# gue-ni/raytracer.glsl

Measured on AMD Instinct MI355X. Metric: Mpaths/s at 1920x1080, 8 bounces, 10k tris, higher is better.
Workload: dtype f32; 1 GPU; C2: 1920x1080, 8 bounces, 10000 triangles + 5 spheres, cube map 256^2, 1 spp/frame progressive, dof=1; parallelism=1 GPU(s), 8-row strips interleaved, gather to rank 0 every frame, frame_batch=1, kernel=4, wf_rays=4, wf_mode=1, wf_chunk=256, wf_early=0, wf_packed=0, mf_sets=4, mf_group_quads=32, mf_chunk_quads=32

## Files before the change

### raytracer.glsl_amd/csrc/rt_scan.hpp

```cpp
#pragma once
#include <type_traits>
#include "rt_mfma.hpp"

#pragma clang fp contract(off)

namespace rt {

typedef uint32_t u32x4 __attribute__((ext_vector_type(4)));
typedef float f32x6 __attribute__((ext_vector_type(6)));

template <bool kMax> __device__ __forceinline__ float half_reduce(float x)
{
    auto op = [](float a, float b) { return kMax ? __builtin_fmaxf(a, b) : __builtin_fminf(a, b); };
    auto dpp = [](float v, auto ctrl) { return __builtin_bit_cast(float, __builtin_amdgcn_update_dpp(0, __builtin_bit_cast(int, v), decltype(ctrl)::value, 0xf, 0xf, false)); };
    x = op(x, dpp(x, std::integral_constant<int, 0xB1>{}));
    x = op(x, dpp(x, std::integral_constant<int, 0x4E>{}));
    x = op(x, dpp(x, std::integral_constant<int, 0x141>{}));
    x = op(x, dpp(x, std::integral_constant<int, 0x140>{}));
    const float r0 = __builtin_bit_cast(float, __builtin_amdgcn_readlane(__builtin_bit_cast(int, x), 0));
    const float r1 = __builtin_bit_cast(float, __builtin_amdgcn_readlane(__builtin_bit_cast(int, x), 16));
    return op(r0, r1);
}
__device__ __forceinline__ float half_max(float x) { return half_reduce<true>(x); }
__device__ __forceinline__ float half_min(float x) { return half_reduce<false>(x); }
template <bool kMax> __device__ __forceinline__ float full_reduce(float x)
{
    auto op = [](float a, float b) { return kMax ? __builtin_fmaxf(a, b) : __builtin_fminf(a, b); };
    auto dpp = [](float v, auto ctrl) { return __builtin_bit_cast(float, __builtin_amdgcn_update_dpp(0, __builtin_bit_cast(int, v), decltype(ctrl)::value, 0xf, 0xf, false)); };
    x = op(x, dpp(x, std::integral_constant<int, 0xB1>{}));
    x = op(x, dpp(x, std::integral_constant<int, 0x4E>{}));
    x = op(x, dpp(x, std::integral_constant<int, 0x141>{}));
    x = op(x, dpp(x, std::integral_constant<int, 0x140>{}));
    auto rl = [&](int l) { return __builtin_bit_cast(float, __builtin_amdgcn_readlane(__builtin_bit_cast(int, x), l)); };
    return op(op(rl(0), rl(16)), op(rl(32), rl(48)));
}

constexpr uint32_t kCullRowWords = 128;
__device__ __forceinline__ void wave_lds_sync() { __builtin_amdgcn_fence(__ATOMIC_ACQ_REL, "wavefront"); __builtin_amdgcn_wave_barrier(); }
__device__ __forceinline__ bool cull_lane(const MfCull &c, bool have, const MfPacket &pk)
{
    bool skip = false, open = false;
    f3 W = mk(0.0f, 0.0f, 0.0f); float L = 0.0f, nz = 0.0f, Wn = 0.0f;
    if (have && c.Nmin > 0.0f) {
        const f3 gq = pk.O - mk(c.cx, c.cy, c.cz);
        L = __builtin_amdgcn_sqrtf(dot3(gq, gq)) * 1.0001f;
        nz = 9.5367431640625e-07f * __builtin_fmaf(c.lmax, pk.On, c.Pw) * 1.01f;
        W = cross3(pk.D, gq);
        Wn = __builtin_amdgcn_sqrtf(dot3(W, W));
        skip = mf_certified_ka(c, pk, gq, L, nz, Wn);
        open = !skip;
    }
    if (__any(open)) { if (open) skip = mf_certified_b(c, pk, W, L, nz, Wn); }
    return skip;
}

__global__ void __launch_bounds__(256) packet_cull_kernel(WaveBuffers wb, const MfCull *__restrict__ cull, uint32_t n_tiles, uint32_t bounce, float ro_add, float sigma_add,
                                                          const MfCull *__restrict__ node, uint32_t node_shift)
{
    __shared__ uint32_t s_row[4][kCullRowWords];
    __shared__ uint32_t s_open[4][64];
    const uint32_t n_rays = wb.counts[bounce];
    const RayQueue qin = (bounce & 1u) ? wb.q[1] : wb.q[0];
    const uint32_t lane = threadIdx.x & 63u, n_gran = (n_rays + 127u) / 128u;
    const float inf = __builtin_inff();
    for (uint32_t g = blockIdx.x * 4u + (threadIdx.x >> 6); g < n_gran; g += gridDim.x * 4u) {
        f3 o[2], dh[2]; bool valid[2]; bool usable = true;
        f3 olo = mk(inf, inf, inf), ohi = mk(-inf, -inf, -inf), dlo = olo, dhi = ohi;
#pragma unroll
        for (int k = 0; k < 2; ++k) {
            const uint32_t slot = g * 128u + (uint32_t)k * 64u + lane;
            valid[k] = slot < n_rays;
            o[k] = mk(0.0f, 0.0f, 0.0f); dh[k] = o[k];
            if (valid[k]) {
                const float4 a = qin.a[slot], b = qin.b[slot];
                o[k] = mk(a.x, a.y, a.z);
                const f3 d = mk(a.w, b.x, b.y);
                const float dd = dot3(d, d), il = __builtin_amdgcn_rsqf(dd), dl = dd * il;
                dh[k] = mk(d.x * il, d.y * il, d.z * il);
                usable &= (dl > 0.0f) && (dl < inf) && (fabsf(o[k].x) < 1e18f) && (fabsf(o[k].y) < 1e18f) && (fabsf(o[k].z) < 1e18f);
                olo = mk(fminf(olo.x, o[k].x), fminf(olo.y, o[k].y), fminf(olo.z, o[k].z)); ohi = mk(fmaxf(ohi.x, o[k].x), fmaxf(ohi.y, o[k].y), fmaxf(ohi.z, o[k].z));
                dlo = mk(fminf(dlo.x, dh[k].x), fminf(dlo.y, dh[k].y), fminf(dlo.z, dh[k].z)); dhi = mk(fmaxf(dhi.x, dh[k].x), fmaxf(dhi.y, dh[k].y), fmaxf(dhi.z, dh[k].z));
            }
        }
        olo = mk(full_reduce<false>(olo.x), full_reduce<false>(olo.y), full_reduce<false>(olo.z)); ohi = mk(full_reduce<true>(ohi.x), full_reduce<true>(ohi.y), full_reduce<true>(ohi.z));
        dlo = mk(full_reduce<false>(dlo.x), full_reduce<false>(dlo.y), full_reduce<false>(dlo.z)); dhi = mk(full_reduce<true>(dhi.x), full_reduce<true>(dhi.y), full_reduce<true>(dhi.z));
        MfPacket pk;
        pk.O = mk(0.5f * olo.x + 0.5f * ohi.x, 0.5f * olo.y + 0.5f * ohi.y, 0.5f * olo.z + 0.5f * ohi.z);
        f3 D = mk(0.5f * dlo.x + 0.5f * dhi.x, 0.5f * dlo.y + 0.5f * dhi.y, 0.5f * dlo.z + 0.5f * dhi.z);
        const float DD = dot3(D, D), iDl = __builtin_amdgcn_rsqf(DD), Dl = DD * iDl;
        pk.D = mk(D.x * iDl, D.y * iDl, D.z * iDl);
        float ro = 0.0f, sigma = 0.0f;
#pragma unroll
        for (int k = 0; k < 2; ++k)
            if (valid[k]) {
                const f3 eo = o[k] - pk.O, ed = dh[k] - pk.D;
                ro = fmaxf(ro, __builtin_amdgcn_sqrtf(dot3(eo, eo))); sigma = fmaxf(sigma, __builtin_amdgcn_sqrtf(dot3(ed, ed)));
            }
        pk.ro = full_reduce<true>(ro) * 1.0001f + 1e-30f + ro_add; pk.sigma = full_reduce<true>(sigma) * 1.0001f + 2e-6f + sigma_add;
        usable = !__any(!usable) && (Dl > 0.25f);
        pk.On = __builtin_amdgcn_sqrtf(dot3(pk.O, pk.O)) * 1.0001f + pk.ro;
        uint32_t *const row = wb.keep + (size_t)g * wb.keep_words;
        if (node_shift) {
            const uint32_t wv = threadIdx.x >> 6, S = 1u << node_shift, n_nodes = (n_tiles + S - 1u) >> node_shift;
            const uint32_t batch_nodes = (kCullRowWords * 32u) >> node_shift;
            const uint32_t grp = min(S, 32u);
            for (uint32_t b0 = 0; b0 < n_nodes; b0 += batch_nodes) {
                const uint32_t tile0 = b0 << node_shift, w0 = tile0 >> 5;
// ... 733 lines not shown
```

### raytracer.glsl_amd/csrc/rt_wavefront.hpp

```cpp
#pragma once
#include "rt_device.hpp"

#pragma clang fp contract(off)

namespace rt {

enum { kScalar = 0, kLds = 1 };
constexpr int kTile = 256;
constexpr int kBoundGroup = 64;

struct RayQueue {
    float4 *a;
    float4 *b;
    float4 *c;
    uint4 *rng;
    uint32_t *pixel;
};

struct WaveBuffers {
    RayQueue q[2];
    uint32_t *counts;
    float4 *sums;
    float4 *cam_a, *cam_b;
    uint4 *pix_rng;
    const float2 *group_bounds;
    unsigned long long *best[2];
    uint2 *cand;
    uint32_t *cand_counts;
    uint32_t cand_region;
    uint32_t *keep;
    uint32_t keep_words;
    uint32_t *items;
    uint32_t *item_counts;
    uint32_t items_stride;
    uint32_t hybrid_div;
    uint32_t *plan_prefix;
    uint32_t plan_stride;
    uint32_t *plan_total;
    unsigned long long *plan_base;
    uint32_t *sched;
    uint32_t sched_stride;
    uint32_t *cand_peak;
    RayQueue qt;
    uint2 *sort_kr;
    uint32_t *sort_hist;
    uint32_t *sort_hist_other;
    uint32_t sort_bits;
    uint32_t sort_ob;
    uint32_t sort_db, sort_T;
    float sort_lo[3], sort_inv_cell[3];
    float sort_in_lo[3], sort_in_hi[3];
    float sort_cen[3], sort_inv_unit;
    uint32_t sort_in_bits, sort_out_bits;
    uint32_t sort_in_order, sort_out_order;
    float4 *batch_rad;
    uint32_t batch_px;
};
constexpr uint32_t kBatchMax = 16u;
constexpr uint32_t kBatchPixelMask = 0x0FFFFFFFu;
struct BatchInfo { uint32_t n; int32_t frames[kBatchMax]; int32_t reset[kBatchMax]; };

struct PathState { f3 o, d, thr, rad; Rng rng; uint32_t pixel; };

typedef float rt_f4v __attribute__((ext_vector_type(4)));
typedef uint32_t rt_u4v __attribute__((ext_vector_type(4)));
typedef uint32_t rt_u2v __attribute__((ext_vector_type(2)));
__device__ __forceinline__ void store_through(float4 *p, float x, float y, float z, float w) { const rt_f4v v = {x, y, z, w}; asm volatile("global_store_dwordx4 %0, %1, off sc0 sc1\n\ts_nop 1" :: "v"(p), "v"(v) : "memory"); }
__device__ __forceinline__ void store_through(uint4 *p, uint32_t x, uint32_t y, uint32_t z, uint32_t w) { const rt_u4v v = {x, y, z, w}; asm volatile("global_store_dwordx4 %0, %1, off sc0 sc1\n\ts_nop 1" :: "v"(p), "v"(v) : "memory"); }
__device__ __forceinline__ void store_through(uint32_t *p, uint32_t x) { asm volatile("global_store_dword %0, %1, off sc0 sc1" :: "v"(p), "v"(x) : "memory"); }
__device__ __forceinline__ void store_through(unsigned long long *p, unsigned long long x) { const rt_u2v v = {(uint32_t)x, (uint32_t)(x >> 32)}; asm volatile("global_store_dwordx2 %0, %1, off sc0 sc1\n\ts_nop 1" :: "v"(p), "v"(v) : "memory"); }

__device__ __forceinline__ void store_ray(const RayQueue &q, uint32_t slot, const PathState &s, bool camera = false)
{
    store_through(q.a + slot, s.o.x, s.o.y, s.o.z, s.d.x);
    store_through(q.b + slot, s.d.y, s.d.z, s.thr.x, s.thr.y);
    if (!camera) store_through(q.c + slot, s.thr.z, s.rad.x, s.rad.y, s.rad.z);
    store_through(q.rng + slot, s.rng.x, s.rng.y, s.rng.z, s.rng.w);
// ... 504 lines not shown
    const float oa[3] = {o.x, o.y, o.z};
    const bool inside = o.x >= wb.sort_in_lo[0] && o.x <= wb.sort_in_hi[0] && o.y >= wb.sort_in_lo[1] && o.y <= wb.sort_in_hi[1] && o.z >= wb.sort_in_lo[2] && o.z <= wb.sort_in_hi[2];
    const uint32_t bits3 = inside ? wb.sort_in_bits : wb.sort_out_bits, order = inside ? wb.sort_in_order : wb.sort_out_order;
    uint32_t c[3], left[3];
#pragma unroll
    for (int a = 0; a < 3; ++a) {
        const uint32_t nb = (bits3 >> (4 * a)) & 15u;
        left[a] = nb;
        if (inside) c[a] = (uint32_t)fminf(fmaxf((oa[a] - wb.sort_lo[a]) * wb.sort_inv_cell[a], 0.0f), (float)((1u << nb) - 1u));
        else {
            const float u = fminf(fabsf(oa[a] - wb.sort_cen[a]) * wb.sort_inv_unit, 1.0e6f);
            const uint32_t j = min(7u, (__float_as_uint(1.0f + u) >> 23) - 127u);
            c[a] = (oa[a] >= wb.sort_cen[a] ? 8u + j : 7u - j) >> (4u - nb);
        }
    }
    uint32_t cell = 0u;
    const uint32_t n = left[0] + left[1] + left[2];
    for (uint32_t i = 0; i < n; ++i) {
        const uint32_t a = (order >> (2u * i)) & 3u;
        const uint32_t l = (a == 0u ? left[0] : a == 1u ? left[1] : left[2]) - 1u;
        const uint32_t v = a == 0u ? c[0] : a == 1u ? c[1] : c[2];
        cell = (cell << 1) | ((v >> l) & 1u);
        left[0] = a == 0u ? l : left[0]; left[1] = a == 1u ? l : left[1]; left[2] = a == 2u ? l : left[2];
    }
    return (dir << (T + 1u)) | (inside ? 0u : 1u << T) | (cell << (T - n));
}

template <bool kCount, bool kSort>
__global__ void __launch_bounds__(256) shade_kernel(SceneView sc, FrameParams P, ImageView im, WaveBuffers wb,
                                                    uint32_t bounce, uint4 *rng_out, Counters *counters)
{
    const uint32_t n_rays = wb.counts[bounce];
    const RayQueue qin = (bounce & 1u) ? wb.q[1] : wb.q[0];
    const RayQueue qout = kSort ? wb.qt : ((bounce & 1u) ? wb.q[0] : wb.q[1]);
    const unsigned long long *best_in = (bounce & 1u) ? wb.best[1] : wb.best[0];
    unsigned long long *best_out = (bounce & 1u) ? wb.best[0] : wb.best[1];
    const bool last_bounce = (bounce + 1u >= P.max_bounce);
    unsigned long long c_env = 0;
    __shared__ uint32_t s_cnt[5];
    for (uint32_t blk = blockIdx.x; blk * 256u < n_rays; blk += gridDim.x) {
    const uint32_t slot = blk * 256u + threadIdx.x;
    const bool valid = slot < n_rays;
    bool alive = false;
    PathState s;
    if (valid) {
        s = load_ray(qin, slot, bounce == 0u);
        const unsigned long long key = best_in[slot];
        Hit h; h.t = kInf; h.material = 0; h.point = h.normal = mk(0.0f, 0.0f, 0.0f);
        const bool hit_sphere = sphere_pass(sc, s.o, s.d, h);
        const bool hit_mesh = key != kNoHitKey;
        if (!hit_sphere && !hit_mesh) {
            f3 bg;
            if (P.use_envmap) { bg = env_lookup(sc, s.d); if (kCount) c_env++; }
            else bg = mk(P.background[0], P.background[1], P.background[2]);
            s.rad = s.rad + bg * s.thr;
        } else {
            const float mesh_t = hit_mesh ? __uint_as_float((uint32_t)(key >> 32)) : kInf;
            if (!(h.t < mesh_t)) {
                const TriPlane pl = sc.tri_planes[(uint32_t)key];
                h.t = mesh_t; h.point = s.o + s.d * mesh_t; h.normal = mk(pl.nx, pl.ny, pl.nz); h.material = pl.material;
            }
            alive = shade_hit(sc, h, s.rng, s.o, s.d, s.thr, s.rad) && !last_bounce;
        }
        if (!alive) finish_path(P, im, wb, s, rng_out);
    }
    const unsigned long long mask = __ballot(alive);
    const int lane = threadIdx.x & 63, wave = threadIdx.x >> 6;
    if (lane == 0) s_cnt[wave] = (uint32_t)__popcll(mask);
    __syncthreads();
    if (threadIdx.x == 0) {
        const uint32_t total = s_cnt[0] + s_cnt[1] + s_cnt[2] + s_cnt[3];
        s_cnt[4] = total ? atomicAdd(&wb.counts[bounce + 1u], total) : 0u;
    }
    __syncthreads();
    if (alive) {
        uint32_t wave_base = s_cnt[4];
        for (int w = 0; w < wave; ++w) wave_base += s_cnt[w];
        const uint32_t out_slot = wave_base + (uint32_t)__popcll(mask & ((1ull << lane) - 1ull));
        if (kSort) {
            const uint32_t key = ray_bin_key(wb, s.o, s.d);
            uint32_t grp_n = 1u, grp_rank = 0u; int grp_leader = lane;
            for (unsigned long long todo = __ballot(1); todo;) {
                const int l = __builtin_ctzll(todo);
                const uint32_t k0 = (uint32_t)__builtin_amdgcn_readlane((int)key, l);
                const unsigned long long m = __ballot(key == k0);
                if (key == k0) { grp_n = (uint32_t)__popcll(m); grp_rank = (uint32_t)__popcll(m & ((1ull << lane) - 1ull)); grp_leader = l; }
                todo &= ~m;
            }
            uint32_t base = 0u;
            if (lane == grp_leader) base = atomicAdd(wb.sort_hist + key, grp_n);
            const uint32_t rank = (uint32_t)__shfl((int)base, grp_leader) + grp_rank;
            store_ray(qout, out_slot, s);
            store_through(reinterpret_cast<unsigned long long *>(wb.sort_kr + out_slot), (unsigned long long)key | ((unsigned long long)rank << 32));
        } else { store_ray(qout, out_slot, s); store_through(best_out + out_slot, kNoHitKey); }
    }
    __syncthreads();
    }
    if (kCount) {
        atomicAdd(&counters->env_lookups, c_env);
        if (blockIdx.x == 0 && threadIdx.x == 0) atomicAdd(&counters->segments, (unsigned long long)n_rays);
    }
}

constexpr uint32_t kSortSeg = 4096;
__global__ void __launch_bounds__(256) sort_sums_kernel(WaveBuffers wb)
{
    __shared__ uint32_t part[4];
    const uint32_t *h = wb.sort_hist + (size_t)blockIdx.x * kSortSeg;
    const uint4 *h4 = reinterpret_cast<const uint4 *>(h);
    uint32_t s = 0;
#pragma unroll
    for (int k = 0; k < 4; ++k) { const uint4 v = h4[k * 256 + threadIdx.x]; s += v.x + v.y + v.z + v.w; }
    for (int off = 32; off > 0; off >>= 1) s += __shfl_xor(s, off);
    if ((threadIdx.x & 63u) == 0u) part[threadIdx.x >> 6] = s;
    __syncthreads();
    if (threadIdx.x == 0) store_through(wb.sort_hist + ((size_t)1u << wb.sort_bits) + blockIdx.x, part[0] + part[1] + part[2] + part[3]);
}
__global__ void __launch_bounds__(256) sort_prefix_kernel(WaveBuffers wb)
{
    __shared__ uint32_t part[4], wsum[4];
    const uint32_t *sums = wb.sort_hist + ((size_t)1u << wb.sort_bits);
    uint32_t before = 0;
    for (uint32_t i = threadIdx.x; i < blockIdx.x; i += 256u) before += sums[i];
    for (int off = 32; off > 0; off >>= 1) before += __shfl_xor(before, off);
    if ((threadIdx.x & 63u) == 0u) part[threadIdx.x >> 6] = before;
    __syncthreads();
    before = part[0] + part[1] + part[2] + part[3];
    uint32_t *h = wb.sort_hist + (size_t)blockIdx.x * kSortSeg + threadIdx.x * 16u;
    uint4 v[4];
#pragma unroll
    for (int k = 0; k < 4; ++k) v[k] = reinterpret_cast<const uint4 *>(h)[k];
    uint32_t c[16] = {v[0].x, v[0].y, v[0].z, v[0].w, v[1].x, v[1].y, v[1].z, v[1].w, v[2].x, v[2].y, v[2].z, v[2].w, v[3].x, v[3].y, v[3].z, v[3].w};
    uint32_t tot = 0;
#pragma unroll
    for (int k = 0; k < 16; ++k) { const uint32_t t = c[k]; c[k] = tot; tot += t; }
    uint32_t inc = tot;
    const uint32_t lane = threadIdx.x & 63u, wave = threadIdx.x >> 6;
    for (int off = 1; off < 64; off <<= 1) { const uint32_t t = __shfl_up(inc, off); if (lane >= (uint32_t)off) inc += t; }
    if (lane == 63u) wsum[wave] = inc;
    __syncthreads();
    uint32_t base = before + inc - tot;
    for (uint32_t w = 0; w < wave; ++w) base += wsum[w];
#pragma unroll
    for (int k = 0; k < 4; ++k) store_through(reinterpret_cast<uint4 *>(h) + k, base + c[4 * k], base + c[4 * k + 1], base + c[4 * k + 2], base + c[4 * k + 3]);
}
__global__ void __launch_bounds__(256) sort_scatter_kernel(WaveBuffers wb, uint32_t bounce)
{
    const uint32_t n_rays = wb.counts[bounce];
    const RayQueue qout = (bounce & 1u) ? wb.q[1] : wb.q[0];
    unsigned long long *best_out = (bounce & 1u) ? wb.best[1] : wb.best[0];
    {
        uint4 *const z = reinterpret_cast<uint4 *>(wb.sort_hist_other);
        const uint32_t n4 = (uint32_t)(((size_t)1u << wb.sort_bits) / 4u);
        for (uint32_t w = blockIdx.x * 256u + threadIdx.x; w < n4; w += gridDim.x * 256u) store_through(z + w, 0u, 0u, 0u, 0u);
    }
    for (uint32_t slot = blockIdx.x * 256u + threadIdx.x; slot < n_rays; slot += gridDim.x * 256u) {
        const uint2 kr = wb.sort_kr[slot];
        const uint32_t to = wb.sort_hist[kr.x] + kr.y;
        const float4 a = wb.qt.a[slot], b = wb.qt.b[slot], c = wb.qt.c[slot];
        const uint4 g = wb.qt.rng[slot];
        const uint32_t px = wb.qt.pixel[slot];
        if (to >= n_rays) { store_through(best_out + slot, kNoHitKey); continue; }
        store_through(qout.a + to, a.x, a.y, a.z, a.w);
        store_through(qout.b + to, b.x, b.y, b.z, b.w);
        store_through(qout.c + to, c.x, c.y, c.z, c.w);
        store_through(qout.rng + to, g.x, g.y, g.z, g.w);
        store_through(qout.pixel + to, px);
        store_through(best_out + slot, kNoHitKey);
    }
}

__global__ void __launch_bounds__(64) group_bounds_kernel(const TriEdges *__restrict__ edges, uint32_t n, float2 *__restrict__ out)
{
    const uint32_t g = blockIdx.x, v = g * kBoundGroup + threadIdx.x;
    float be = 0.0f, bm = 0.0f;
    if (v < n) { be = edges[v].bound_e; bm = edges[v].bound_m; }
    bool bad = !(be == be) || !(bm == bm);
#pragma unroll
    for (int off = 32; off > 0; off >>= 1) {
        be = fmaxf(be, __shfl_xor(be, off));
        bm = fmaxf(bm, __shfl_xor(bm, off));
    }
    if (__any(bad)) { be = __builtin_nanf(""); bm = __builtin_nanf(""); }
    if (threadIdx.x == 0) out[g] = make_float2(be, bm);
}

}
```

### raytracer.glsl_amd/csrc/rtgl_amd.hip

```cpp
#include <hip/hip_runtime.h>
#include <algorithm>
#include <cmath>
#include <cstdio>
#include <cstring>
#include <string>
#include <vector>
#include <map>
#include <mutex>
#include <thread>
#include <condition_variable>
#include <memory>

#include "../../include/rtgl_amd.h"
#include "rt_device.hpp"
#include "rt_wavefront.hpp"
#include "rt_mfma.hpp"
#include "rt_scan.hpp"

#pragma clang fp contract(off)

using namespace rt;


__global__ void __launch_bounds__(256) prepare_triangles_kernel(const float4 *__restrict__ vertices,
// ... 132 lines not shown
    std::vector<uint8_t> h_meshes, h_nodes, h_vertices;
    uint32_t n_meshes = 0, n_nodes = 0, n_vec4 = 0;

    SphereRec *d_spheres = nullptr; uint32_t n_spheres = 0;
    MaterialRec *d_materials = nullptr; uint32_t n_materials = 0;
    float4 *d_vertices = nullptr;
    uint32_t *d_sphere_visits = nullptr; uint32_t n_sphere_visits = 0;
    TriEdges *d_edges = nullptr; TriPlane *d_planes = nullptr; uint32_t n_tri_visits = 0;
    TriEdges *d_edges_s = nullptr; TriPlane *d_planes_s = nullptr;
    uint8_t *d_env = nullptr; int env_w = 0, env_h = 0, env_c = 0, env_faces = 0;
    float4 *d_image_own = nullptr, *d_image = nullptr;
    uint4 *d_rng = nullptr;
    Counters *d_counters = nullptr;
    uchar4 *d_u8 = nullptr;

    float2 *d_group_bounds = nullptr;
    MfGroup *d_mf_groups = nullptr; MfCull *d_mf_cull = nullptr; MfCull *d_mf_cull_node = nullptr; uint32_t cull_node_shift = 0; uint4 *d_mf_A = nullptr; uint32_t *d_mf_order = nullptr; uint32_t n_mf_groups = 0, mf_group_quads = 32; uint32_t *d_dbg_log = nullptr;
    void *d_wave = nullptr; size_t wave_capacity = 0; bool wave_multi = false;
    uint32_t *d_counts = nullptr; uint32_t counts_capacity = 0;
    uint32_t *h_counts = nullptr;
    hipEvent_t counts_ev = nullptr; bool counts_pending = false, counts_valid = false;
    bool timing_this_frame = false; uint32_t timing_frame_counter = 0;
    int kernel_in_use = -1;
    int n_cus = 256;
    uint2 *d_items = nullptr; size_t items_capacity = 0;
    uint32_t *d_sched = nullptr; size_t sched_capacity = 0;
    uint32_t *d_keep = nullptr; size_t keep_capacity = 0;
    uint32_t *d_keep0 = nullptr; size_t keep0_capacity = 0; bool keep0_valid = false; FrameParams keep0_params{}; uint32_t keep0_n0 = 0, keep0_words = 0; uint64_t keep0_scene = 0;
    uint64_t scene_version = 0;
    void *d_plan = nullptr; size_t plan_capacity = 0;
    void *d_stage = nullptr; size_t stage_capacity = 0;
    uint32_t *d_sort_hist = nullptr; uint32_t sort_bits_alloc = 0;
    int sort_set = 0; uint32_t sort_set_bits = 0; bool sort_sets_clean = false;
    float mesh_lo[3] = {0.0f, 0.0f, 0.0f}, mesh_hi[3] = {0.0f, 0.0f, 0.0f}, mesh_ext = 0.0f;
    uint2 *d_cand = nullptr; uint32_t cand_regions = 0, cand_region_pairs = 0, cand_region_target = 0; bool cand_fixed = false;
    bool solo_attr_set = false;
    bool group_explicit = false;
    bool kernel_explicit = false;
    uint32_t counts_n0 = 0, counts_len = 0;
    std::vector<uint32_t> est_counts;
    WaveBuffers wb{};

    std::vector<rtgl_context *> parts;
    std::vector<hipEvent_t> part_done;
    hipEvent_t gather_done = nullptr;
    std::vector<std::unique_ptr<PartWorker>> workers;
    bool gathered = false, peer_copy = true;

    std::vector<FrameParams> pending;
    float4 *d_batch_rad = nullptr; size_t batch_capacity = 0;
    uint32_t last_batch_frames = 1;
    bool tris_dirty = false, visits_dirty = false;
    FrameParams params{};
    bool have_params = false;
    int opt_kernel = RTGL_KERNEL_WAVEFRONT_MFMA_SOLO, opt_rng_state = 0, opt_counters = 0, opt_kernel_timing = 0, opt_wf_rays = 4, opt_wf_mode = kLds, opt_wf_chunk = 256, opt_wf_early = 0, opt_wf_packed = 0, opt_mf_chunk_quads = 32, opt_mf_group_quads = 32, opt_cull = 3, opt_sort_min_rays = 131072, opt_scan_waves = 0, opt_scan_dynamic = 0, opt_debug_skip_exact = 0, opt_frame_batch = 1;
};

static int fail(rtgl_context *ctx, int code, const std::string &msg)
{
    if (ctx) ctx->error = msg; else g_create_error = msg;
    return code;
}
#define HIPCHK(ctx, expr) do { hipError_t e_ = (expr); if (e_ != hipSuccess) \
    return fail(ctx, RTGL_ERR_DEVICE, std::string(#expr) + ": " + hipGetErrorString(e_)); } while (0)

template <typename T>
// ... 69 lines not shown
    *out = nullptr;
    if (width <= 0 || height <= 0 || world < 1 || rank < 0 || rank >= world || strip_rows <= 0 || (strip_rows % 8) != 0)
        return fail(nullptr, RTGL_ERR_INVALID, "rtgl_create: bad size / tiling arguments");
    int ndev = 0;
    if (hipGetDeviceCount(&ndev) != hipSuccess || ndev <= 0)
        return fail(nullptr, RTGL_ERR_NO_DEVICE, "no HIP device visible (this library has no CPU path)");
    if (device < 0 || device >= ndev) return fail(nullptr, RTGL_ERR_INVALID, "device ordinal out of range");
    rtgl_context *ctx = new rtgl_context();
    ctx->device = device; ctx->width = width; ctx->height = height;
    ctx->rank = rank; ctx->world = world; ctx->strip_rows = strip_rows;
    ctx->local_rows = local_rows_for(height, rank, world, strip_rows);
    auto bail = [&](int code) { g_create_error = ctx->error; rtgl_destroy(ctx); return code; };
#define CCHK(expr) do { hipError_t e_ = (expr); if (e_ != hipSuccess) { \
    ctx->error = std::string(#expr) + ": " + hipGetErrorString(e_); return bail(RTGL_ERR_DEVICE); } } while (0)
    CCHK(hipSetDevice(device));
    { hipDeviceProp_t prop; if (hipGetDeviceProperties(&prop, device) == hipSuccess && prop.multiProcessorCount > 0) ctx->n_cus = prop.multiProcessorCount; }
    CCHK(acquire_device_stream(device, &ctx->own_stream, &ctx->own_stream_shared));
    ctx->stream = ctx->own_stream;
    register_ctx_stream(ctx, device, ctx->stream);
    CCHK(hipEventCreate(&ctx->ev0));
    CCHK(hipEventCreate(&ctx->ev1));
    size_t img_bytes = (size_t)std::max(ctx->local_rows, 1) * width * sizeof(float4);
    CCHK(hipMalloc((void **)&ctx->d_image_own, img_bytes));
    CCHK(hipMemsetAsync(ctx->d_image_own, 0, img_bytes, ctx->stream));
    ctx->d_image = ctx->d_image_own;
    CCHK(hipMalloc((void **)&ctx->d_counters, 64));
    CCHK(hipMemsetAsync(ctx->d_counters, 0, 64, ctx->stream));
    CCHK(hipStreamSynchronize(ctx->stream));
#undef CCHK
    if (const char *k = getenv("RTGL_AMD_KERNEL")) { const int v = atoi(k); if (v >= RTGL_KERNEL_MEGA && v <= RTGL_KERNEL_WAVEFRONT_MFMA_SOLO && v != RTGL_KERNEL_REMOVED_3) { ctx->opt_kernel = v; ctx->kernel_explicit = true; } }
    if (const char *k = getenv("RTGL_AMD_SCAN_WAVES")) { const int v = atoi(k); if (v >= 0 && v <= 2) ctx->opt_scan_waves = v; }
    if (const char *k = getenv("RTGL_AMD_FRAME_BATCH")) { const int v = atoi(k); if (v >= 1 && v <= (int)kBatchMax) ctx->opt_frame_batch = v; }
    if (const char *k = getenv("RTGL_AMD_SCAN_DYNAMIC")) { const int v = atoi(k); if (v >= 0 && v <= 4) ctx->opt_scan_dynamic = v; }
    *out = ctx;
    return RTGL_OK;
}

static int flush_pending_noexcept(rtgl_context *ctx);
extern "C" int rtgl_create(rtgl_context **out, int width, int height, int device)
{
    return rtgl_create_tiled(out, width, height, device, 0, 1, 8);
}

extern "C" void rtgl_destroy(rtgl_context *ctx)
{
    if (!ctx) return;
    if (!ctx->pending.empty() && hipSetDevice(ctx->device) == hipSuccess && flush_pending_noexcept(ctx) != RTGL_OK)
        fprintf(stderr, "rtgl_destroy: %zu batched frame(s) could not be submitted: %s\n", ctx->pending.size(), ctx->error.c_str());
    unregister_ctx_stream(ctx);
    for (auto &w : ctx->workers) {
        { std::lock_guard<std::mutex> lk(w->m); w->state = PartWorker::kQuit; }
        w->cv.notify_all();
        if (w->th.joinable()) w->th.join();
    }
    ctx->workers.clear();
    for (rtgl_context *part : ctx->parts) rtgl_destroy(part);
    ctx->parts.clear();
    (void)hipSetDevice(ctx->device);
    for (hipEvent_t e : ctx->part_done) (void)hipEventDestroy(e);
    if (ctx->gather_done) (void)hipEventDestroy(ctx->gather_done);
    if (ctx->stream) (void)hipStreamSynchronize(ctx->stream);
#ifdef RT_SOLO_STAMPS
    if (ctx->d_dbg_log) {
        unsigned long long h[16 * 64];
        if (hipMemcpy(h, ctx->d_dbg_log, sizeof h, hipMemcpyDeviceToHost) == hipSuccess)
            for (int b = 0; b < 64 && h[16 * b + 8]; ++b) {
// ... 463 lines not shown
    const size_t local_px = (size_t)std::max(ctx->local_rows, 1) * ctx->width;
    if (ctx->opt_kernel == RTGL_KERNEL_WAVEFRONT_MFMA_SOLO) {
        const uint32_t need_regions = solo_regions(ctx);
        if (!ctx->cand_region_target) ctx->cand_region_target = std::max<uint32_t>(4096u, (uint32_t)std::min<uint64_t>(((uint64_t)n0 + need_regions - 1) / need_regions, 0xFFFFFFF0u));
        if (!ctx->d_cand || need_regions > ctx->cand_regions || ctx->cand_region_target > ctx->cand_region_pairs) {
            if (ctx->d_cand) { HIPCHK(ctx, hipFree(ctx->d_cand)); ctx->d_cand = nullptr; }
            ctx->cand_regions = need_regions; ctx->cand_region_pairs = ctx->cand_region_target;
            HIPCHK(ctx, hipMalloc((void **)&ctx->d_cand, ((size_t)need_regions * ctx->cand_region_pairs) * sizeof(uint2) + (size_t)need_regions * sizeof(uint32_t) + 256));
        }
        {
            const uint32_t real_quads = std::min(ctx->n_mf_groups * ctx->mf_group_quads, (ctx->n_tri_visits + (uint32_t)kMfQuadTris - 1) / (uint32_t)kMfQuadTris);
            ctx->wb.keep_words = std::max(1u, (real_quads * (uint32_t)kMfQuadTiles + 31u) / 32u);
            const size_t need = ((size_t)n0 / 128 + 16) * ctx->wb.keep_words;
            if (ctx->keep_capacity < need) {
                if (ctx->d_keep) { HIPCHK(ctx, hipFree(ctx->d_keep)); ctx->d_keep = nullptr; }
                HIPCHK(ctx, hipMalloc((void **)&ctx->d_keep, need * sizeof(uint32_t)));
                ctx->keep_capacity = need;
            }
        }
        ctx->wb.keep = ctx->d_keep;
        {
            ctx->wb.sched_stride = std::max<uint32_t>((uint32_t)ctx->n_cus, solo_chunks(ctx));
            const size_t need = (size_t)(max_bounce + 2) * ctx->wb.sched_stride;
            if (ctx->sched_capacity < need) {
                if (ctx->d_sched) { HIPCHK(ctx, hipFree(ctx->d_sched)); ctx->d_sched = nullptr; }
                HIPCHK(ctx, hipMalloc((void **)&ctx->d_sched, need * sizeof(uint32_t)));
                ctx->sched_capacity = need;
            }
            ctx->wb.sched = ctx->d_sched;
        }
        if (ctx->opt_cull == 3) {
            if (ctx->stage_capacity < n0) {
                if (ctx->d_stage) { HIPCHK(ctx, hipFree(ctx->d_stage)); ctx->d_stage = nullptr; }
                HIPCHK(ctx, hipMalloc(&ctx->d_stage, (size_t)n0 * 76 + 1024));
                ctx->stage_capacity = n0;
            }
            uint8_t *p = (uint8_t *)ctx->d_stage;
            const size_t cap = ctx->stage_capacity;
            ctx->wb.qt.a = (float4 *)p; p += cap * 16; ctx->wb.qt.b = (float4 *)p; p += cap * 16; ctx->wb.qt.c = (float4 *)p; p += cap * 16;
            ctx->wb.qt.rng = (uint4 *)p; p += cap * 16; ctx->wb.sort_kr = (uint2 *)p; p += cap * 8; ctx->wb.qt.pixel = (uint32_t *)p;
            ctx->wb.sort_ob = n0 > (12u << 20) ? 5u : 4u;
            if (const char *e = getenv("RTGL_AMD_SORT_OB")) { const int v = atoi(e); if (v >= 1 && v <= 5) ctx->wb.sort_ob = (uint32_t)v; }
            ctx->wb.sort_db = 4u;
            if (const char *e = getenv("RTGL_AMD_SORT_DB")) { const int v = atoi(e); if (v >= 2 && v <= 6) ctx->wb.sort_db = (uint32_t)v; }
            ctx->wb.sort_bits = 8u + 3u * ctx->wb.sort_ob;
            ctx->wb.sort_T = ctx->wb.sort_bits - 1u - 2u * ctx->wb.sort_db;
            if (ctx->sort_bits_alloc < ctx->wb.sort_bits) {
                if (ctx->d_sort_hist) { HIPCHK(ctx, hipFree(ctx->d_sort_hist)); ctx->d_sort_hist = nullptr; }
                const size_t bins = (size_t)1 << ctx->wb.sort_bits;
                HIPCHK(ctx, hipMalloc((void **)&ctx->d_sort_hist, 2 * (bins + bins / kSortSeg) * sizeof(uint32_t)));
                ctx->sort_bits_alloc = ctx->wb.sort_bits; ctx->sort_sets_clean = false;
            }
            ctx->wb.sort_hist = ctx->d_sort_hist; ctx->wb.sort_hist_other = ctx->d_sort_hist;
            set_bin_cells(ctx);
        }
        ctx->wb.hybrid_div = 3u;
        if (const char *e = getenv("RTGL_AMD_HYBRID_DIV")) { const int v = atoi(e); if (v >= 1 && v <= 64) ctx->wb.hybrid_div = (uint32_t)v; }
        ctx->wb.items = reinterpret_cast<uint32_t *>(ctx->d_items); ctx->wb.item_counts = reinterpret_cast<uint32_t *>(ctx->d_items);
        ctx->wb.cand = ctx->d_cand;
        ctx->wb.cand_counts = reinterpret_cast<uint32_t *>(ctx->d_cand + (size_t)ctx->cand_regions * ctx->cand_region_pairs);
        ctx->wb.cand_region = ctx->cand_region_pairs;
        if (const char *cc = getenv("RTGL_DEBUG_CAND_CAP")) { ctx->wb.cand_region = std::min<uint32_t>(ctx->wb.cand_region, (uint32_t)atoi(cc)); ctx->cand_fixed = true; }
    }
    if (ctx->wave_capacity < n0 || (multi_sample && !ctx->wave_multi)) {
        if (ctx->d_wave) { HIPCHK(ctx, hipFree(ctx->d_wave)); ctx->d_wave = nullptr; }
        size_t q_bytes = (size_t)n0 * (68 + 8), bytes = 2 * q_bytes + 1024 + (multi_sample ? local_px * 64 : 0);
        HIPCHK(ctx, hipMalloc(&ctx->d_wave, bytes));
        ctx->wave_capacity = n0; ctx->wave_multi = multi_sample;
        uint8_t *p = (uint8_t *)ctx->d_wave;
        for (int q = 0; q < 2; ++q) {
            ctx->wb.q[q].a = (float4 *)p; p += (size_t)n0 * 16;
            ctx->wb.q[q].b = (float4 *)p; p += (size_t)n0 * 16;
            ctx->wb.q[q].c = (float4 *)p; p += (size_t)n0 * 16;
// ... 104 lines not shown
    MfView mf{ctx->d_mf_groups, ctx->n_mf_groups, gq, n_quads, ctx->d_mf_A, ctx->d_dbg_log, ctx->d_mf_cull, ctx->d_edges_s, ctx->d_planes_s, ctx->d_mf_order};
    if (!ctx->solo_attr_set) {
        for (const void *fn : {reinterpret_cast<const void *>(&scan_solo_kernel<false, 1, 0>), reinterpret_cast<const void *>(&scan_solo_kernel<true, 1, 0>),
                               reinterpret_cast<const void *>(&scan_solo_kernel<false, 2, 0>), reinterpret_cast<const void *>(&scan_solo_kernel<true, 2, 0>),
                               reinterpret_cast<const void *>(&scan_solo_kernel<false, 1, 1>), reinterpret_cast<const void *>(&scan_solo_kernel<true, 1, 1>),
                               reinterpret_cast<const void *>(&scan_solo_kernel<false, 2, 1>), reinterpret_cast<const void *>(&scan_solo_kernel<true, 2, 1>),
                               reinterpret_cast<const void *>(&scan_solo_kernel<false, 1, 2>), reinterpret_cast<const void *>(&scan_solo_kernel<true, 1, 2>),
                               reinterpret_cast<const void *>(&scan_solo_kernel<false, 2, 2>), reinterpret_cast<const void *>(&scan_solo_kernel<true, 2, 2>),
                               reinterpret_cast<const void *>(&scan_solo_kernel<false, 1, 3>), reinterpret_cast<const void *>(&scan_solo_kernel<true, 1, 3>),
                               reinterpret_cast<const void *>(&scan_solo_kernel<false, 2, 3>), reinterpret_cast<const void *>(&scan_solo_kernel<true, 2, 3>)}) {
            hipFuncAttributes fattr;
            HIPCHK(ctx, hipFuncGetAttributes(&fattr, fn));
            HIPCHK(ctx, hipFuncSetAttribute(fn, hipFuncAttributeMaxDynamicSharedMemorySize, (int)(160 * 1024 - fattr.sharedSizeBytes)));
        }
        ctx->solo_attr_set = true;
    }

    if (cull) {
        float ro_add = 0.0f, sigma_add = 0.0f;
        bool have_bits = false;
        if (bounce == 0 && cam && camera_keep_widening(*cam, &ro_add, &sigma_add) && !getenv("RTGL_AMD_NO_CAMERA_KEEP")) {
            const size_t need = ((size_t)n0 / 128 + 16) * ctx->wb.keep_words;
            if (ctx->keep0_capacity < need) {
                if (ctx->d_keep0) { HIPCHK(ctx, hipFree(ctx->d_keep0)); ctx->d_keep0 = nullptr; }
                HIPCHK(ctx, hipMalloc((void **)&ctx->d_keep0, need * sizeof(uint32_t)));
                ctx->keep0_capacity = need; ctx->keep0_valid = false;
            }
            have_bits = ctx->keep0_valid && ctx->keep0_n0 == n0 && ctx->keep0_words == ctx->wb.keep_words && ctx->keep0_scene == ctx->scene_version && same_camera(ctx->keep0_params, *cam);
            ctx->wb.keep = ctx->d_keep0;
            if (!have_bits) { ctx->keep0_valid = true; ctx->keep0_n0 = n0; ctx->keep0_words = ctx->wb.keep_words; ctx->keep0_scene = ctx->scene_version; ctx->keep0_params = *cam; }
        } else { ctx->wb.keep = ctx->d_keep; ro_add = sigma_add = 0.0f; }
        if (!have_bits)
        hipLaunchKernelGGL(packet_cull_kernel, dim3(std::max(1u, std::min((est_gran + 3u) / 4u, 8192u))), dim3(256), 0, ctx->stream, ctx->wb, ctx->d_mf_cull, real_quads * (uint32_t)kMfQuadTiles, bounce, ro_add, sigma_add,
                           ctx->d_mf_cull_node, ctx->d_mf_cull_node ? ctx->cull_node_shift : 0u);
        if (dist == 2) {
            const uint32_t stride = n0 / Cfg::kRaysPerWave + 1u;
            const size_t off_tot = (((size_t)chunks * stride * sizeof(uint32_t)) + 255) & ~(size_t)255, off_base = (off_tot + (size_t)chunks * sizeof(uint32_t) + 255) & ~(size_t)255;
            const size_t need = off_base + ((size_t)chunks + 1) * sizeof(unsigned long long);
            if (ctx->plan_capacity < need) {
                if (ctx->d_plan) { HIPCHK(ctx, hipFree(ctx->d_plan)); ctx->d_plan = nullptr; }
                HIPCHK(ctx, hipMalloc(&ctx->d_plan, need));
                ctx->plan_capacity = need;
            }
            ctx->wb.plan_prefix = reinterpret_cast<uint32_t *>(ctx->d_plan); ctx->wb.plan_stride = stride;
            ctx->wb.plan_total = reinterpret_cast<uint32_t *>(reinterpret_cast<uint8_t *>(ctx->d_plan) + off_tot);
            ctx->wb.plan_base = reinterpret_cast<unsigned long long *>(reinterpret_cast<uint8_t *>(ctx->d_plan) + off_base);
            if (ctx->opt_counters) hipLaunchKernelGGL(scan_plan_kernel<true>, dim3(chunks), dim3(256), 0, ctx->stream, ctx->wb, bounce, chunk_quads, real_quads, ctx->d_counters);
            else hipLaunchKernelGGL(scan_plan_kernel<false>, dim3(chunks), dim3(256), 0, ctx->stream, ctx->wb, bounce, chunk_quads, real_quads, ctx->d_counters);
            hipLaunchKernelGGL(scan_plan_base_kernel, dim3(1), dim3(64), 0, ctx->stream, ctx->wb, chunks);
        }
        if (dynamic) {
        const uint32_t stride = n0 / Cfg::kRaysPerWave + 1u;
        const size_t head = ((size_t)ctx->wb.sched_stride * sizeof(uint32_t) + 255) & ~(size_t)255, need = head + (size_t)chunks * stride * sizeof(uint32_t);
        if (ctx->items_capacity < need) {
            if (ctx->d_items) { HIPCHK(ctx, hipFree(ctx->d_items)); ctx->d_items = nullptr; }
            HIPCHK(ctx, hipMalloc((void **)&ctx->d_items, need));
            ctx->items_capacity = need;
        }
        ctx->wb.item_counts = reinterpret_cast<uint32_t *>(ctx->d_items);
        ctx->wb.items = reinterpret_cast<uint32_t *>(reinterpret_cast<uint8_t *>(ctx->d_items) + head);
        ctx->wb.items_stride = stride;
        HIPCHK(ctx, hipMemsetAsync(ctx->wb.item_counts, 0, (size_t)chunks * sizeof(uint32_t), ctx->stream));
        const dim3 igrid(std::max(1u, std::min((est_gran + 255u) / 256u, 1024u)), chunks);
        if (ctx->opt_counters) hipLaunchKernelGGL(cull_items_kernel<true>, igrid, dim3(256), 0, ctx->stream, ctx->wb, bounce, chunk_quads, real_quads, ctx->d_counters);
        else hipLaunchKernelGGL(cull_items_kernel<false>, igrid, dim3(256), 0, ctx->stream, ctx->wb, bounce, chunk_quads, real_quads, ctx->d_counters);
        }
    }
// ... 45 lines not shown
                } else if (sc.n_tri_visits > 0) {
                    kev_mark(ctx);
                    switch (key) {
                    case 1: launch_intersect<1, kScalar>(ctx, sc, n0, b); break;
                    case 2: launch_intersect<2, kScalar>(ctx, sc, n0, b); break;
                    case 4: launch_intersect<4, kScalar>(ctx, sc, n0, b); break;
                    case 8: launch_intersect<8, kScalar>(ctx, sc, n0, b); break;
                    case 11: launch_intersect<1, kLds>(ctx, sc, n0, b); break;
                    case 12: launch_intersect<2, kLds>(ctx, sc, n0, b); break;
                    case 14: launch_intersect<4, kLds>(ctx, sc, n0, b); break;
                    case 18: launch_intersect<8, kLds>(ctx, sc, n0, b); break;
                    default: return fail(ctx, RTGL_ERR_STATE, "unsupported wf_mode / wf_rays combination");
                    }
                    kev_mark(ctx);
                }
                const dim3 shade_grid((estimate_rays(ctx, n0, b) + 255) / 256);
                const uint32_t est_next = estimate_rays(ctx, n0, b + 1u);
                const bool bin_next = ctx->opt_kernel == RTGL_KERNEL_WAVEFRONT_MFMA_SOLO && ctx->opt_cull == 3 && sc.n_tri_visits > 0 && b + 1u < P.max_bounce
                                      && est_next >= (uint32_t)ctx->opt_sort_min_rays;
                if (bin_next) {
                    const size_t bins = (size_t)1 << ctx->wb.sort_bits, set_words = bins + bins / kSortSeg;
                    if (!ctx->sort_sets_clean || ctx->sort_set_bits != ctx->wb.sort_bits) {
                        HIPCHK(ctx, hipMemsetAsync(ctx->d_sort_hist, 0, 2 * set_words * sizeof(uint32_t), ctx->stream));
                        ctx->sort_set = 0; ctx->sort_set_bits = ctx->wb.sort_bits;
                    }
                    ctx->sort_sets_clean = false;
                    if (getenv("RTGL_AMD_HIST_FILL")) HIPCHK(ctx, hipMemsetAsync(ctx->d_sort_hist + (size_t)ctx->sort_set * set_words, 0, bins * sizeof(uint32_t), ctx->stream));
                    ctx->wb.sort_hist = ctx->d_sort_hist + (size_t)ctx->sort_set * set_words;
                    ctx->wb.sort_hist_other = ctx->d_sort_hist + (size_t)(ctx->sort_set ^ 1) * set_words;
                    if (ctx->opt_counters) hipLaunchKernelGGL((shade_kernel<true, true>), shade_grid, dim3(256), 0, ctx->stream, sc, P, im, ctx->wb, b, rng_out, ctx->d_counters);
                    else hipLaunchKernelGGL((shade_kernel<false, true>), shade_grid, dim3(256), 0, ctx->stream, sc, P, im, ctx->wb, b, rng_out, ctx->d_counters);
                    hipLaunchKernelGGL(sort_sums_kernel, dim3((unsigned)(bins / kSortSeg)), dim3(256), 0, ctx->stream, ctx->wb);
                    hipLaunchKernelGGL(sort_prefix_kernel, dim3((unsigned)(bins / kSortSeg)), dim3(256), 0, ctx->stream, ctx->wb);
                    hipLaunchKernelGGL(sort_scatter_kernel, dim3(std::max(1u, std::min((est_next + 255u) / 256u, 16384u))), dim3(256), 0, ctx->stream, ctx->wb, b + 1u);
                    HIPCHK(ctx, hipGetLastError());
                    ctx->sort_set ^= 1; ctx->sort_sets_clean = true;
                } else if (ctx->opt_counters)
                    hipLaunchKernelGGL((shade_kernel<true, false>), shade_grid, dim3(256), 0, ctx->stream, sc, P, im, ctx->wb, b, rng_out, ctx->d_counters);
                else
                    hipLaunchKernelGGL((shade_kernel<false, false>), shade_grid, dim3(256), 0, ctx->stream, sc, P, im, ctx->wb, b, rng_out, ctx->d_counters);
                binned = bin_next;
                continue;
            }
            kev_mark(ctx);
            switch (key) {
            case 1: launch_bounce<1, kScalar>(ctx, sc, P, im, n0, b, rng_out); break;
            case 2: launch_bounce<2, kScalar>(ctx, sc, P, im, n0, b, rng_out); break;
            case 4: launch_bounce<4, kScalar>(ctx, sc, P, im, n0, b, rng_out); break;
            case 11: launch_bounce<1, kLds>(ctx, sc, P, im, n0, b, rng_out); break;
            case 12: launch_bounce<2, kLds>(ctx, sc, P, im, n0, b, rng_out); break;
            case 14: launch_bounce<4, kLds>(ctx, sc, P, im, n0, b, rng_out); break;
            default: return fail(ctx, RTGL_ERR_STATE, "unsupported wf_mode / wf_rays combination");
            }
            kev_mark(ctx);
        }
        HIPCHK(ctx, hipGetLastError());
    }
    if (P.samples > 1u) {
        hipLaunchKernelGGL(resolve_kernel, gen_grid, dim3(256), 0, ctx->stream, P, im, ctx->wb);
        HIPCHK(ctx, hipGetLastError());
    }
    if (B > 1) {
        BatchInfo bi{};
        bi.n = B;
        for (uint32_t f = 0; f < B; ++f) { bi.frames[f] = frames[f].frames; bi.reset[f] = frames[f].reset_flag; }
        hipLaunchKernelGGL(resolve_batch_kernel, gen_grid, dim3(256), 0, ctx->stream, im, ctx->wb, bi);
        HIPCHK(ctx, hipGetLastError());
// ... 450 lines not shown
```

Before: 854.8 Mpaths/s.

## Replace ray scatter pass with index placement and gather inside packet cull

Shade now writes sorted-path rays as packed 64-byte records through LDS into an interleaved stage buffer. A new placement kernel then writes only a source index per destination slot, instead of scattering full ray records. The packet cull kernel gathers each ray from stage and writes it into the input queue while it reads it, which removes one full read/write pass over the ray data. This adds an LDS buffer to shade, indirect reads in cull, and a waves_per_eu hint on the cull kernel that may restrict its register budget.

```diff
diff --git a/raytracer.glsl_amd/csrc/rt_scan.hpp b/raytracer.glsl_amd/csrc/rt_scan.hpp
--- a/raytracer.glsl_amd/csrc/rt_scan.hpp
+++ b/raytracer.glsl_amd/csrc/rt_scan.hpp
@@ -54,8 +54,8 @@
     return skip;
 }
 
-__global__ void __launch_bounds__(256) packet_cull_kernel(WaveBuffers wb, const MfCull *__restrict__ cull, uint32_t n_tiles, uint32_t bounce, float ro_add, float sigma_add,
-                                                          const MfCull *__restrict__ node, uint32_t node_shift)
+__global__ void __launch_bounds__(256) __attribute__((amdgpu_waves_per_eu(5))) packet_cull_kernel(WaveBuffers wb, const MfCull *__restrict__ cull, uint32_t n_tiles, uint32_t bounce, float ro_add, float sigma_add,
+                                                          const MfCull *__restrict__ node, uint32_t node_shift, uint32_t gather)
 {
     __shared__ uint32_t s_row[4][kCullRowWords];
     __shared__ uint32_t s_open[4][64];
@@ -72,7 +72,20 @@
             valid[k] = slot < n_rays;
             o[k] = mk(0.0f, 0.0f, 0.0f); dh[k] = o[k];
             if (valid[k]) {
-                const float4 a = qin.a[slot], b = qin.b[slot];
+                float4 a, b;
+                const uint32_t from = gather ? wb.sort_src[slot] : n_rays;
+                if (from < n_rays) {
+                    const float4 *const rec = wb.stage + 4u * from;
+                    a = rec[0]; b = rec[1];
+                    const float4 c = rec[2];
+                    const uint4 r = *reinterpret_cast<const uint4 *>(rec + 3);
+                    const uint32_t px = wb.stage_pixel[from];
+                    store_through(qin.a + slot, a.x, a.y, a.z, a.w);
+                    store_through(qin.b + slot, b.x, b.y, b.z, b.w);
+                    store_through(qin.c + slot, c.x, c.y, c.z, c.w);
+                    store_through(qin.rng + slot, r.x, r.y, r.z, r.w);
+                    store_through(qin.pixel + slot, px);
+                } else { a = qin.a[slot]; b = qin.b[slot]; }
                 o[k] = mk(a.x, a.y, a.z);
                 const f3 d = mk(a.w, b.x, b.y);
                 const float dd = dot3(d, d), il = __builtin_amdgcn_rsqf(dd), dl = dd * il;
diff --git a/raytracer.glsl_amd/csrc/rt_wavefront.hpp b/raytracer.glsl_amd/csrc/rt_wavefront.hpp
--- a/raytracer.glsl_amd/csrc/rt_wavefront.hpp
+++ b/raytracer.glsl_amd/csrc/rt_wavefront.hpp
@@ -41,8 +41,10 @@
     uint32_t *sched;
     uint32_t sched_stride;
     uint32_t *cand_peak;
-    RayQueue qt;
+    float4 *stage;
+    uint32_t *stage_pixel;
     uint2 *sort_kr;
+    uint32_t *sort_src;
     uint32_t *sort_hist;
     uint32_t *sort_hist_other;
     uint32_t sort_bits;
@@ -613,12 +615,13 @@
 {
     const uint32_t n_rays = wb.counts[bounce];
     const RayQueue qin = (bounce & 1u) ? wb.q[1] : wb.q[0];
-    const RayQueue qout = kSort ? wb.qt : ((bounce & 1u) ? wb.q[0] : wb.q[1]);
+    const RayQueue qout = (bounce & 1u) ? wb.q[0] : wb.q[1];
     const unsigned long long *best_in = (bounce & 1u) ? wb.best[1] : wb.best[0];
     unsigned long long *best_out = (bounce & 1u) ? wb.best[0] : wb.best[1];
     const bool last_bounce = (bounce + 1u >= P.max_bounce);
     unsigned long long c_env = 0;
     __shared__ uint32_t s_cnt[5];
+    __shared__ float4 s_rec[kSort ? 4 * 64 * 4 : 1];
     for (uint32_t blk = blockIdx.x; blk * 256u < n_rays; blk += gridDim.x) {
     const uint32_t slot = blk * 256u + threadIdx.x;
     const bool valid = slot < n_rays;
@@ -654,9 +657,9 @@
         s_cnt[4] = total ? atomicAdd(&wb.counts[bounce + 1u], total) : 0u;
     }
     __syncthreads();
+    uint32_t wave_base = s_cnt[4];
+    for (int w = 0; w < wave; ++w) wave_base += s_cnt[w];
     if (alive) {
-        uint32_t wave_base = s_cnt[4];
-        for (int w = 0; w < wave; ++w) wave_base += s_cnt[w];
         const uint32_t out_slot = wave_base + (uint32_t)__popcll(mask & ((1ull << lane) - 1ull));
         if (kSort) {
             const uint32_t key = ray_bin_key(wb, s.o, s.d);
@@ -670,10 +673,23 @@
             }
             uint32_t base = 0u;
             if (lane == grp_leader) base = atomicAdd(wb.sort_hist + key, grp_n);
+            float4 *const r = s_rec + (wave * 64u + (out_slot - wave_base)) * 4u;
+            r[0] = make_float4(s.o.x, s.o.y, s.o.z, s.d.x); r[1] = make_float4(s.d.y, s.d.z, s.thr.x, s.thr.y);
+            r[2] = make_float4(s.thr.z, s.rad.x, s.rad.y, s.rad.z);
+            r[3] = make_float4(__uint_as_float(s.rng.x), __uint_as_float(s.rng.y), __uint_as_float(s.rng.z), __uint_as_float(s.rng.w));
+            store_through(wb.stage_pixel + out_slot, s.pixel);
             const uint32_t rank = (uint32_t)__shfl((int)base, grp_leader) + grp_rank;
-            store_ray(qout, out_slot, s);
             store_through(reinterpret_cast<unsigned long long *>(wb.sort_kr + out_slot), (unsigned long long)key | ((unsigned long long)rank << 32));
         } else { store_ray(qout, out_slot, s); store_through(best_out + out_slot, kNoHitKey); }
+    }
+    if (kSort) {
+        __builtin_amdgcn_fence(__ATOMIC_ACQ_REL, "wavefront"); __builtin_amdgcn_wave_barrier();
+        const uint32_t parts = 4u * (uint32_t)__popcll(mask);
+#pragma unroll
+        for (uint32_t k = 0; k < 4u; ++k) {
+            const uint32_t i = k * 64u + lane;
+            if (i < parts) { const float4 v = s_rec[wave * 256u + i]; store_through(wb.stage + 4u * wave_base + i, v.x, v.y, v.z, v.w); }
+        }
     }
     __syncthreads();
     }
@@ -725,22 +741,37 @@
 #pragma unroll
     for (int k = 0; k < 4; ++k) store_through(reinterpret_cast<uint4 *>(h) + k, base + c[4 * k], base + c[4 * k + 1], base + c[4 * k + 2], base + c[4 * k + 3]);
 }
+__device__ __forceinline__ void sort_zero_other(const WaveBuffers &wb)
+{
+    uint4 *const z = reinterpret_cast<uint4 *>(wb.sort_hist_other);
+    const uint32_t n4 = (uint32_t)(((size_t)1u << wb.sort_bits) / 4u);
+    for (uint32_t w = blockIdx.x * 256u + threadIdx.x; w < n4; w += gridDim.x * 256u) store_through(z + w, 0u, 0u, 0u, 0u);
+}
+__global__ void __launch_bounds__(256) sort_place_kernel(WaveBuffers wb, uint32_t bounce)
+{
+    const uint32_t n_rays = wb.counts[bounce];
+    unsigned long long *best_out = (bounce & 1u) ? wb.best[1] : wb.best[0];
+    sort_zero_other(wb);
+    for (uint32_t slot = blockIdx.x * 256u + threadIdx.x; slot < n_rays; slot += gridDim.x * 256u) {
+        const uint2 kr = wb.sort_kr[slot];
+        const uint32_t to = wb.sort_hist[kr.x] + kr.y;
+        if (to < n_rays) store_through(wb.sort_src + to, slot);
+        store_through(best_out + slot, kNoHitKey);
+    }
+}
 __global__ void __launch_bounds__(256) sort_scatter_kernel(WaveBuffers wb, uint32_t bounce)
 {
     const uint32_t n_rays = wb.counts[bounce];
     const RayQueue qout = (bounce & 1u) ? wb.q[1] : wb.q[0];
     unsigned long long *best_out = (bounce & 1u) ? wb.best[1] : wb.best[0];
-    {
-        uint4 *const z = reinterpret_cast<uint4 *>(wb.sort_hist_other);
-        const uint32_t n4 = (uint32_t)(((size_t)1u << wb.sort_bits) / 4u);
-        for (uint32_t w = blockIdx.x * 256u + threadIdx.x; w < n4; w += gridDim.x * 256u) store_through(z + w, 0u, 0u, 0u, 0u);
-    }
+    sort_zero_other(wb);
     for (uint32_t slot = blockIdx.x * 256u + threadIdx.x; slot < n_rays; slot += gridDim.x * 256u) {
         const uint2 kr = wb.sort_kr[slot];
         const uint32_t to = wb.sort_hist[kr.x] + kr.y;
-        const float4 a = wb.qt.a[slot], b = wb.qt.b[slot], c = wb.qt.c[slot];
-        const uint4 g = wb.qt.rng[slot];
-        const uint32_t px = wb.qt.pixel[slot];
+        const float4 *const r = wb.stage + 4u * slot;
+        const float4 a = r[0], b = r[1], c = r[2];
+        const uint4 g = *reinterpret_cast<const uint4 *>(r + 3);
+        const uint32_t px = wb.stage_pixel[slot];
         if (to >= n_rays) { store_through(best_out + slot, kNoHitKey); continue; }
         store_through(qout.a + to, a.x, a.y, a.z, a.w);
         store_through(qout.b + to, b.x, b.y, b.z, b.w);
diff --git a/raytracer.glsl_amd/csrc/rtgl_amd.hip b/raytracer.glsl_amd/csrc/rtgl_amd.hip
--- a/raytracer.glsl_amd/csrc/rtgl_amd.hip
+++ b/raytracer.glsl_amd/csrc/rtgl_amd.hip
@@ -188,6 +188,7 @@
     void *d_stage = nullptr; size_t stage_capacity = 0;
     uint32_t *d_sort_hist = nullptr; uint32_t sort_bits_alloc = 0;
     int sort_set = 0; uint32_t sort_set_bits = 0; bool sort_sets_clean = false;
+    int opt_sort_move = 1;
     float mesh_lo[3] = {0.0f, 0.0f, 0.0f}, mesh_hi[3] = {0.0f, 0.0f, 0.0f}, mesh_ext = 0.0f;
     uint2 *d_cand = nullptr; uint32_t cand_regions = 0, cand_region_pairs = 0, cand_region_target = 0; bool cand_fixed = false;
     bool solo_attr_set = false;
@@ -323,6 +324,7 @@
     if (const char *k = getenv("RTGL_AMD_SCAN_WAVES")) { const int v = atoi(k); if (v >= 0 && v <= 2) ctx->opt_scan_waves = v; }
     if (const char *k = getenv("RTGL_AMD_FRAME_BATCH")) { const int v = atoi(k); if (v >= 1 && v <= (int)kBatchMax) ctx->opt_frame_batch = v; }
     if (const char *k = getenv("RTGL_AMD_SCAN_DYNAMIC")) { const int v = atoi(k); if (v >= 0 && v <= 4) ctx->opt_scan_dynamic = v; }
+    if (const char *k = getenv("RTGL_AMD_SORT_MOVE")) { const int v = atoi(k); if (v == 0 || v == 1) ctx->opt_sort_move = v; }
     *out = ctx;
     return RTGL_OK;
 }
@@ -852,13 +854,13 @@
         if (ctx->opt_cull == 3) {
             if (ctx->stage_capacity < n0) {
                 if (ctx->d_stage) { HIPCHK(ctx, hipFree(ctx->d_stage)); ctx->d_stage = nullptr; }
-                HIPCHK(ctx, hipMalloc(&ctx->d_stage, (size_t)n0 * 76 + 1024));
+                HIPCHK(ctx, hipMalloc(&ctx->d_stage, (size_t)n0 * 80 + 1024));
                 ctx->stage_capacity = n0;
             }
             uint8_t *p = (uint8_t *)ctx->d_stage;
             const size_t cap = ctx->stage_capacity;
-            ctx->wb.qt.a = (float4 *)p; p += cap * 16; ctx->wb.qt.b = (float4 *)p; p += cap * 16; ctx->wb.qt.c = (float4 *)p; p += cap * 16;
-            ctx->wb.qt.rng = (uint4 *)p; p += cap * 16; ctx->wb.sort_kr = (uint2 *)p; p += cap * 8; ctx->wb.qt.pixel = (uint32_t *)p;
+            ctx->wb.stage = (float4 *)p; p += cap * 64; ctx->wb.sort_kr = (uint2 *)p; p += cap * 8; ctx->wb.stage_pixel = (uint32_t *)p; p += cap * 4;
+            ctx->wb.sort_src = (uint32_t *)p;
             ctx->wb.sort_ob = n0 > (12u << 20) ? 5u : 4u;
             if (const char *e = getenv("RTGL_AMD_SORT_OB")) { const int v = atoi(e); if (v >= 1 && v <= 5) ctx->wb.sort_ob = (uint32_t)v; }
             ctx->wb.sort_db = 4u;
@@ -1029,7 +1031,7 @@
         } else { ctx->wb.keep = ctx->d_keep; ro_add = sigma_add = 0.0f; }
         if (!have_bits)
         hipLaunchKernelGGL(packet_cull_kernel, dim3(std::max(1u, std::min((est_gran + 3u) / 4u, 8192u))), dim3(256), 0, ctx->stream, ctx->wb, ctx->d_mf_cull, real_quads * (uint32_t)kMfQuadTiles, bounce, ro_add, sigma_add,
-                           ctx->d_mf_cull_node, ctx->d_mf_cull_node ? ctx->cull_node_shift : 0u);
+                           ctx->d_mf_cull_node, ctx->d_mf_cull_node ? ctx->cull_node_shift : 0u, (uint32_t)(binned && ctx->opt_sort_move == 1));
         if (dist == 2) {
             const uint32_t stride = n0 / Cfg::kRaysPerWave + 1u;
             const size_t off_tot = (((size_t)chunks * stride * sizeof(uint32_t)) + 255) & ~(size_t)255, off_base = (off_tot + (size_t)chunks * sizeof(uint32_t) + 255) & ~(size_t)255;
@@ -1141,7 +1143,8 @@
                     else hipLaunchKernelGGL((shade_kernel<false, true>), shade_grid, dim3(256), 0, ctx->stream, sc, P, im, ctx->wb, b, rng_out, ctx->d_counters);
                     hipLaunchKernelGGL(sort_sums_kernel, dim3((unsigned)(bins / kSortSeg)), dim3(256), 0, ctx->stream, ctx->wb);
                     hipLaunchKernelGGL(sort_prefix_kernel, dim3((unsigned)(bins / kSortSeg)), dim3(256), 0, ctx->stream, ctx->wb);
-                    hipLaunchKernelGGL(sort_scatter_kernel, dim3(std::max(1u, std::min((est_next + 255u) / 256u, 16384u))), dim3(256), 0, ctx->stream, ctx->wb, b + 1u);
+                    if (ctx->opt_sort_move == 1) hipLaunchKernelGGL(sort_place_kernel, dim3(std::max(1u, std::min((est_next + 255u) / 256u, 16384u))), dim3(256), 0, ctx->stream, ctx->wb, b + 1u);
+                    else hipLaunchKernelGGL(sort_scatter_kernel, dim3(std::max(1u, std::min((est_next + 255u) / 256u, 16384u))), dim3(256), 0, ctx->stream, ctx->wb, b + 1u);
                     HIPCHK(ctx, hipGetLastError());
                     ctx->sort_set ^= 1; ctx->sort_sets_clean = true;
                 } else if (ctx->opt_counters)
```

Result: faster. 884.5 Mpaths/s, median of 6 (+3.5%).
